# banyancomputer/hot-proofs-blake3-circom

Hardware: AMD Instinct MI355X
Metric: BLAKE3-compression witnesses/sec (higher is better)
Workload: dtype u32

## Files before the change

hot-proofs-blake3-circom_amd/build.py:

```python
import os, shutil, subprocess, sys

PKG = os.path.dirname(os.path.abspath(__file__))
ROOT = os.path.dirname(PKG)
CSRC = os.path.join(PKG, "csrc")
LIB = os.path.join(PKG, "libb3wit.so")
NAPI = os.path.join(PKG, "js", "b3wit_napi.node")
ARCH = "gfx950"


def _newer(target, sources):
    if not os.path.exists(target):
        return True
    t = os.path.getmtime(target)
    return any(os.path.getmtime(s) > t for s in sources)


def _run(cmd, **kw):
    print("+", " ".join(cmd), flush=True)
    subprocess.check_call(cmd, **kw)


def hipcc():
    for c in (os.environ.get("HIPCC"), shutil.which("hipcc"), "/opt/rocm/bin/hipcc"):
        if c and os.path.exists(c):
            return c
    raise RuntimeError("hipcc not found")


def build_lib(force=False, extra_flags=()):
    from concurrent.futures import ThreadPoolExecutor
    names = ("b3w_kernels.hip", "b3w_exact.hip", "b3w_plan.hip", "b3w_bao.hip", "b3w_placement.hip", "b3w_commit.hip", "b3w_r1cs.hip", "b3w_r1cs_walk.hip", "b3w_r1cs_host.cpp", "b3w_hostcomm.cpp",
             "b3w_ctx.cpp", "b3w_bodies.cpp", "b3w_wtns.cpp", "b3w_r1cs_api.cpp", "b3w_commit_api.cpp", "b3w_comm.cpp", "b3w_chain.cpp")
    srcs = [os.path.join(CSRC, f) for f in names]
    hdrs = [os.path.join(CSRC, f) for f in sorted(os.listdir(CSRC)) if f.endswith((".h", ".inc"))] + \
        [os.path.join(ROOT, "include", "b3wit.h")]
    objdir = os.path.join(PKG, "build")
    os.makedirs(objdir, exist_ok=True)
    if os.environ.get("B3W_BUILD_DIAG") == "1":
        extra_flags = (*extra_flags, "-DB3W_R1CS_DIAG")
    flags = [f"--offload-arch={ARCH}", "-O3", "-std=c++17", "-fPIC", "-x", "hip", "-Wall", "-Wno-unused-function", *extra_flags]
    jobs = []
    for src in srcs:
        obj = os.path.join(objdir, os.path.basename(src) + ".o")
        if force or extra_flags or _newer(obj, [src] + hdrs):
            jobs.append([hipcc(), *flags, "-c", src, "-o", obj])
    if jobs:
        with ThreadPoolExecutor(max_workers=min(len(jobs), os.cpu_count() or 1)) as ex:
            list(ex.map(_run, jobs))
    objs = [os.path.join(objdir, os.path.basename(src) + ".o") for src in srcs]
    if jobs or _newer(LIB, objs):
        _run([hipcc(), f"--offload-arch={ARCH}", "-fPIC", "-shared", "-o", LIB, *objs, "-ldl", "-lrt", "-lpthread"])
    return LIB


def build_oracle(force=False):
    so = os.path.join(ROOT, "oracle", "libb3w_oracle.so")
    if force or _newer(so, [os.path.join(ROOT, "oracle", "b3w_oracle.c")]):
        _run(["make", "-C", os.path.join(ROOT, "oracle")])
    return so


def build_napi(force=False):
    src = os.path.join(PKG, "js", "b3wit_napi.cc")
    if not os.path.exists(src):
        return None
    inc = "/usr/include/node"
    if not os.path.exists(os.path.join(inc, "node_api.h")):
        print("node_api.h not found; skipping N-API addon", file=sys.stderr)
        return None
    if force or _newer(NAPI, [src, os.path.join(ROOT, "include", "b3wit.h")]):
        _run(["g++", "-O2", "-std=c++17", "-fPIC", "-shared", "-DNODE_GYP_MODULE_NAME=b3wit_napi", "-I", inc,
              "-I", os.path.join(ROOT, "include"), "-o", NAPI, src, "-ldl"])
# ... 12 lines not shown
```

hot-proofs-blake3-circom_amd/csrc/b3w_ctx.cpp:

```cpp
#include "b3w_internal.h"
#include "b3w_layout_tables.inc"
#include "b3w_trace_tables.inc"

namespace {

struct Sha256 {
  uint32_t h[8];
  uint8_t buf[64];
  uint64_t len = 0;
  size_t fill = 0;
  Sha256() {
    static const uint32_t init[8] = {0x6a09e667, 0xbb67ae85, 0x3c6ef372, 0xa54ff53a, 0x510e527f, 0x9b05688c, 0x1f83d9ab, 0x5be0cd19};
    memcpy(h, init, sizeof h);
  }
  static uint32_t ror(uint32_t x, int r) { return (x >> r) | (x << (32 - r)); }
  void block(const uint8_t *p) {
    static const uint32_t K[64] = {
        0x428a2f98, 0x71374491, 0xb5c0fbcf, 0xe9b5dba5, 0x3956c25b, 0x59f111f1, 0x923f82a4, 0xab1c5ed5, 0xd807aa98, 0x12835b01,
        0x243185be, 0x550c7dc3, 0x72be5d74, 0x80deb1fe, 0x9bdc06a7, 0xc19bf174, 0xe49b69c1, 0xefbe4786, 0x0fc19dc6, 0x240ca1cc,
        0x2de92c6f, 0x4a7484aa, 0x5cb0a9dc, 0x76f988da, 0x983e5152, 0xa831c66d, 0xb00327c8, 0xbf597fc7, 0xc6e00bf3, 0xd5a79147,
        0x06ca6351, 0x14292967, 0x27b70a85, 0x2e1b2138, 0x4d2c6dfc, 0x53380d13, 0x650a7354, 0x766a0abb, 0x81c2c92e, 0x92722c85,
        0xa2bfe8a1, 0xa81a664b, 0xc24b8b70, 0xc76c51a3, 0xd192e819, 0xd6990624, 0xf40e3585, 0x106aa070, 0x19a4c116, 0x1e376c08,
        0x2748774c, 0x34b0bcb5, 0x391c0cb3, 0x4ed8aa4a, 0x5b9cca4f, 0x682e6ff3, 0x748f82ee, 0x78a5636f, 0x84c87814, 0x8cc70208,
        0x90befffa, 0xa4506ceb, 0xbef9a3f7, 0xc67178f2};
// ... 207 lines not shown
  return buf;
}

}

bool b3w_int_build_slot_table(const CircuitDesc &c, std::vector<uint32_t> &table, std::string &err) { return build_slot_table(c, table, err); }

namespace {
int32_t ensure_scratch(b3w_ctx *ctx) {
  if (ctx->d_scratch) return B3W_OK;
  ctx->scratch_cap = B3W_SWEEP_CHUNK;
  hipError_t e = hipMalloc((void **)&ctx->d_scratch, (size_t)ctx->scratch_cap * ctx->desc.lds_words * 4);
  if (e != hipSuccess) { ctx->scratch_cap = 0; return hip_fail(ctx, e, "hipMalloc(sweep scratch)"); }
  return B3W_OK;
}

void set_inputs(b3w_ctx *ctx) {
  struct Def { const char *name; uint32_t count; };
  static const Def comp[] = {{"h", 8}, {"m", 16}, {"t", 2}, {"b", 1}, {"d", 1}};
  static const Def nova[] = {{"n_blocks", 1}, {"block_count", 1}, {"h", 8}, {"chunk_idx_low", 1}, {"chunk_idx_high", 1},
                             {"leaf_depth", 1}, {"total_depth", 1}, {"depth", 1}, {"m", 16}, {"b", 1}};
  const Def *d = ctx->desc.kind == B3W_KIND_COMP ? comp : nova;
  const int nd = ctx->desc.kind == B3W_KIND_COMP ? 5 : 10;
  uint32_t off = 0;
  for (int i = 0; i < nd; i++) {
    ctx->inputs.push_back({d[i].name, d[i].count, off, fnv1a64(d[i].name)});
    off += d[i].count;
  }
}
}

int b3w_int_default_variant(const b3w_ctx *ctx, uint32_t n, const uint8_t *d_bodies, uint64_t pitch) {
  const bool comp = ctx->desc.kind == B3W_KIND_COMP, nova2 = ctx->desc.kind == B3W_KIND_NOVA_O2;
  const bool fillable = ctx->fill_ok && !(reinterpret_cast<uintptr_t>(d_bodies) & 31) && !(pitch & 31) && pitch < (1ull << 30) &&
                        (uint64_t)n * pitch + (1ull << 20) < (1ull << 37);
  if (fillable && comp && n >= 128 && (n <= 3072 || !b3w_place_is_mixed(d_bodies))) return B3W_VARIANT_REGIONFILL;
  if (fillable && nova2 && (b3w_place_is_mixed(d_bodies) ? n >= 768 && n <= 2560 : n >= 512)) return B3W_VARIANT_REGIONFILL;
  if (n <= 2560) return B3W_VARIANT_SLICED + (n <= (comp ? 32u : 8u) ? 64 : n <= 96 ? 32 : n <= 192 ? 16 : n <= 768 ? 8 : 4);
  if (comp) return n <= 6144 ? 0 : 8;
  if (nova2) return n <= 3072 ? 0 : n <= 32768 ? 3 : 4;
  return 0;
}

extern "C" {

uint32_t b3w_abi_version(void) { return (1u << 16) | 1u; }

int32_t b3w_identify_wasm(const uint8_t *code, size_t len) {
  if (!code) return B3W_CIRCUIT_UNKNOWN;
  Sha256 s;
  s.update(code, len);
  uint8_t dg[32];
  s.final(dg);
  char hex[65];
  for (int i = 0; i < 32; i++) snprintf(hex + 2 * i, 3, "%02x", dg[i]);
  for (int c = 0; c < 4; c++) if (!strcmp(hex, WASM_SHA256[c])) return c;
  return B3W_CIRCUIT_UNKNOWN;
}

int32_t b3w_create(int32_t circuit, int32_t device, b3w_ctx **out) {
  if (!out || circuit < 0 || circuit > 3) return B3W_E_BAD_ARGUMENT;
  *out = nullptr;
  int ndev = 0;
  if (hipGetDeviceCount(&ndev) != hipSuccess || ndev <= 0 || device < 0 || device >= ndev) return B3W_E_NO_DEVICE;
  b3w_ctx *ctx = new b3w_ctx;
  ctx->circuit = circuit;
  ctx->desc = CIRCUITS[circuit];
  ctx->device = device;
// ... 166 lines not shown
uint32_t b3w_public_words(const b3w_ctx *ctx) { return ctx ? ctx->desc.npub : 0; }

int32_t b3w_last_error(const b3w_ctx *ctx, char *buf, size_t len) {
  if (!ctx || !buf || !len) return B3W_E_BAD_ARGUMENT;
  snprintf(buf, len, "%s", ctx->last_error.c_str());
  return B3W_OK;
}

int32_t b3w_write_wtns_header(const b3w_ctx *ctx, uint8_t out[76]) {
  if (!ctx || !out) return B3W_E_BAD_ARGUMENT;
  uint32_t w[19];
  memcpy(&w[0], "wtns", 4);
  w[1] = 2; w[2] = 2;
  w[3] = 1; w[4] = 8 + 32; w[5] = 0;
  w[6] = 32;
  memcpy(&w[7], ctx->desc.prime, 32);
  w[15] = ctx->desc.nwit;
  const uint64_t len = 32ull * ctx->desc.nwit;
  w[16] = 2; w[17] = (uint32_t)len; w[18] = (uint32_t)(len >> 32);
  memcpy(out, w, 76);
  return B3W_OK;
}

int32_t b3w_batch_run_device(b3w_ctx *ctx, const uint32_t *d_records, uint32_t n, uint8_t *d_bodies, uint64_t pitch,
                             uint32_t *d_public, int32_t *d_status, void *stream) {
  if (!ctx || !d_records || !d_bodies) return B3W_E_BAD_ARGUMENT;
  const uint64_t body = 32ull * ctx->desc.nwit;
  if (pitch == 0) pitch = body;
  if (pitch < body || (pitch & 31)) { ctx->last_error = "pitch must be >= witness_size*32 and a multiple of 32"; return B3W_E_BAD_ARGUMENT; }
  if (reinterpret_cast<uintptr_t>(d_bodies) & 15) { ctx->last_error = "d_bodies must be 16-byte aligned"; return B3W_E_BAD_ARGUMENT; }
  ON_DEVICE(ctx);
  int variant = ctx->variant;
  if (ctx->variant_auto || (ctx->variant_tuned && n <= 2560)) variant = b3w_int_default_variant(ctx, n, d_bodies, pitch);
  if (variant >= B3W_VARIANT_REGIONFILL && !ctx->fill_ok) { ctx->last_error = "the fill-ordered variants (200, 201) exist for the compression circuit and the nova O2 builds"; return B3W_E_BAD_ARGUMENT; }
  int rc = b3w_launch_batch(ctx->desc.kind, variant, d_records, n, d_bodies, pitch, ctx->d_table, ctx->desc.nwit,
                            d_public, d_status, ctx->d_aux, ctx->d_scratch, ctx->scratch_cap, (hipStream_t)stream);
  if (rc == 0) return B3W_OK;
  if (rc == -5) { ctx->last_error = "the sweep and fill-ordered paths need 32-byte aligned bodies and pitch < 2^30"; return B3W_E_BAD_ARGUMENT; }
  if (rc < 0) { ctx->last_error = "no kernel for this circuit kind / variant"; return B3W_E_BAD_ARGUMENT; }
  return hip_fail(ctx, (hipError_t)rc, "kernel launch");
}

int32_t b3w_batch_verify_device(b3w_ctx *ctx, const uint8_t *d_bodies, uint32_t n, uint64_t pitch, uint32_t *d_mismatch,
                                void *stream) {
  if (!ctx || !d_bodies || !d_mismatch) return B3W_E_BAD_ARGUMENT;
  if (!ctx->d_in_slots) { ctx->last_error = "this circuit's layout does not keep every input as a slot"; return B3W_E_BAD_ARGUMENT; }
  const uint64_t body = 32ull * ctx->desc.nwit;
  if (pitch == 0) pitch = body;
  if (pitch < body || (pitch & 31) || (reinterpret_cast<uintptr_t>(d_bodies) & 15)) {
    ctx->last_error = "pitch must be >= witness_size*32 and a multiple of 32, bodies 16-byte aligned";
    return B3W_E_BAD_ARGUMENT;
  }
  ON_DEVICE(ctx);
  int rc = b3w_launch_verify(ctx->desc.kind, ctx->d_in_slots, n, d_bodies, pitch, ctx->d_table, ctx->desc.nwit, d_mismatch,
                             ctx->d_aux, (hipStream_t)stream);
  return rc ? hip_fail(ctx, (hipError_t)rc, "verify launch") : B3W_OK;
}

int32_t b3w_batch_autotune_device(b3w_ctx *ctx, const uint32_t *d_records, uint32_t n, uint8_t *d_bodies, uint64_t pitch,
                                  uint32_t *d_public, int32_t *d_status, void *stream, int32_t *chosen_variant,
                                  float *chosen_ms) {
  if (!ctx || !d_records || !d_bodies || !n) return B3W_E_BAD_ARGUMENT;
  ON_DEVICE(ctx);
  int32_t rc;
  if (n <= 2560 && (ctx->variant_auto || ctx->variant_tuned)) {
    float ms = 0;
    rc = B3W_OK;
    for (int w = 0; w < 2 && rc == B3W_OK; w++) rc = b3w_batch_run_device(ctx, d_records, n, d_bodies, pitch, d_public, d_status, stream);
    if (rc == B3W_OK) rc = b3w_batch_time_device(ctx, d_records, n, d_bodies, pitch, d_public, d_status, stream, 5, &ms);
    if (rc) return rc;
    if (chosen_variant) *chosen_variant = b3w_int_default_variant(ctx, n, d_bodies, pitch ? pitch : 32ull * ctx->desc.nwit);
    if (chosen_ms) *chosen_ms = ms;
    return B3W_OK;
  }
  rc = ensure_scratch(ctx);
  if (rc) return rc;
  const int candidates[6] = {0, ctx->desc.kind == B3W_KIND_COMP ? (n > 6144 ? 8 : 3) : ctx->desc.kind == B3W_KIND_NOVA_O2 ? 3 : 0, B3W_VARIANT_SWEEP,
                             ctx->fill_ok ? B3W_VARIANT_REGIONFILL : 0, ctx->desc.kind == B3W_KIND_NOVA_O2 && n >= 16384 ? 4 : 0,
                             ctx->fill_ok ? B3W_VARIANT_REGIONFILL_LIGHT : 0};
  int best = ctx->variant;
  float best_ms = 1e30f;
  const int saved = ctx->variant;
  const bool saved_auto = ctx->variant_auto;
  ctx->variant_auto = false;
  float cand_ms[6] = {1e30f, 1e30f, 1e30f, 1e30f, 1e30f, 1e30f};
  for (int round = 0; round < 2; round++) {
    for (int ci = 0; ci < 6; ci++) {
      const int c = candidates[ci];
      if (ci > 0 && c == candidates[0]) continue;
      if (round > 0 && cand_ms[ci] >= 1e30f) continue;
      ctx->variant = c;
      float ms = 0;
      rc = B3W_OK;
      for (int w = 0; w < 2 && rc == B3W_OK; w++)
        rc = b3w_batch_run_device(ctx, d_records, n, d_bodies, pitch, d_public, d_status, stream);
      if (rc == B3W_OK) rc = b3w_batch_time_device(ctx, d_records, n, d_bodies, pitch, d_public, d_status, stream, n <= 8192 ? 20 : 5, &ms);
      if (rc == B3W_E_BAD_ARGUMENT) continue;
      if (rc) { ctx->variant = saved; ctx->variant_auto = saved_auto; return rc; }
      if (ms < cand_ms[ci]) cand_ms[ci] = ms;
    }
  }
  for (int ci = 0; ci < 6; ci++)
    if (cand_ms[ci] < best_ms) { best_ms = cand_ms[ci]; best = candidates[ci]; }
  if (best_ms >= 1e30f) { ctx->variant = saved; ctx->variant_auto = saved_auto; return B3W_E_BAD_ARGUMENT; }
  ctx->variant = best;
  ctx->variant_tuned = true;
  if (chosen_variant) *chosen_variant = best;
  if (chosen_ms) *chosen_ms = best_ms;
  return B3W_OK;
}

int32_t b3w_batch_time_device(b3w_ctx *ctx, const uint32_t *d_records, uint32_t n, uint8_t *d_bodies, uint64_t pitch,
                              uint32_t *d_public, int32_t *d_status, void *stream, uint32_t iters, float *avg_ms) {
  if (!ctx || !avg_ms || !iters) return B3W_E_BAD_ARGUMENT;
  ON_DEVICE(ctx);
  hipEvent_t e0 = nullptr, e1 = nullptr;
  hipError_t e = hipEventCreate(&e0);
  if (e == hipSuccess) e = hipEventCreate(&e1);
  if (e == hipSuccess) e = hipEventRecord(e0, (hipStream_t)stream);
  int32_t rc = B3W_OK;
  for (uint32_t i = 0; i < iters && e == hipSuccess && rc == B3W_OK; i++)
    rc = b3w_batch_run_device(ctx, d_records, n, d_bodies, pitch, d_public, d_status, stream);
  float ms = 0;
  if (e == hipSuccess && rc == B3W_OK) e = hipEventRecord(e1, (hipStream_t)stream);
  if (e == hipSuccess && rc == B3W_OK) e = hipEventSynchronize(e1);
  if (e == hipSuccess && rc == B3W_OK) e = hipEventElapsedTime(&ms, e0, e1);
  if (e0) (void)hipEventDestroy(e0);
  if (e1) (void)hipEventDestroy(e1);
  if (rc) return rc;
  if (e != hipSuccess) return hip_fail(ctx, e, "timing events");
  *avg_ms = ms / iters;
  return B3W_OK;
}

static int32_t calc_witness_run(b3w_ctx *ctx, const std::vector<uint32_t> &rec, const std::vector<uint8_t> &fe, bool canonical,
                                uint8_t *out_body) {
  const CircuitDesc &d = ctx->desc;
// ... 70 lines not shown
```

hot-proofs-blake3-circom_amd/csrc/b3w_kernels.h:

```cpp
#pragma once
#include <hip/hip_runtime_api.h>
#include <stdint.h>

#define B3W_VARIANT_SWEEP 100
#define B3W_VARIANT_SLICED 20
#define B3W_VARIANT_REGIONFILL 200
#define B3W_VARIANT_REGIONFILL_LIGHT 201
#define B3W_REGIONFILL_GRID 256
#define B3W_AUX_WIDE_SLOTS (16 + 8 * 2048)
#define B3W_AUX_LINE_COUNTS (B3W_AUX_WIDE_SLOTS + 68)
#define B3W_AUX_LINE_LISTS (B3W_AUX_LINE_COUNTS + 4)
#define B3W_LINE_LIST_MAX 160
#define B3W_AUX_ALIAS_COUNT (B3W_AUX_LINE_LISTS + 2 * 4 * B3W_LINE_LIST_MAX)
#define B3W_AUX_ALIAS_LIST (B3W_AUX_ALIAS_COUNT + 1)
#define B3W_ALIAS_MAX 192
#define B3W_SWEEP_GRID 256
#define B3W_SWEEP_LOGC 13
#define B3W_SWEEP_CHUNK (1u << B3W_SWEEP_LOGC)

extern "C" int b3w_launch_batch(int kind, int variant, const uint32_t *d_recs, uint32_t n, uint8_t *d_out,
                                uint64_t pitch, const uint32_t *d_table, uint32_t nwit, uint32_t *d_pub,
                                int32_t *d_status, const void *d_aux, uint32_t *d_scratch, uint32_t scratch_cap,
                                hipStream_t stream);

extern "C" int b3w_launch_exact(int nova, const uint32_t *d_inputs, const uint32_t *d_prime, const uint32_t *d_table,
                                uint32_t nwit, uint8_t *d_out, uint32_t *d_status, hipStream_t stream);

extern "C" uint32_t b3w_plan_path_len(uint64_t chunk, uint64_t nchunks);
extern "C" int b3w_launch_plan_leaves(const uint8_t *d_pre, uint64_t total_len, uint64_t first_chunk, uint32_t nlocal,
                                      uint64_t nchunks, uint32_t *d_recs, uint32_t *d_chunk_cv, hipStream_t stream);
extern "C" int b3w_launch_plan_merge(const uint32_t *d_left, const uint32_t *d_right, uint32_t stride_words, uint64_t npairs,
                                     uint32_t root, uint32_t *d_parents, hipStream_t stream);
extern "C" int b3w_launch_plan_parents(const uint32_t *d_levels, uint64_t nchunks, uint64_t first_chunk, uint32_t nlocal,
                                       uint32_t last_chunk_blocks, uint32_t *d_recs, hipStream_t stream);
extern "C" uint32_t b3w_plan_tree_first_level(uint64_t nchunks);
extern "C" int b3w_launch_plan_tree(uint32_t *d_levels, uint64_t nchunks, uint32_t l0, uint32_t *d_root, uint64_t first_chunk, uint32_t plan_nlocal,
                                    uint32_t last_chunk_blocks, uint32_t *d_recs, hipStream_t stream);
extern "C" uint64_t b3w_plan_parent_row(uint64_t chunk, uint64_t nchunks);
extern "C" int b3w_plan_path_provable(uint64_t chunk, uint64_t nchunks);
extern "C" int b3w_launch_pack_hout(const uint32_t *d_pub, uint64_t row0, uint64_t count, uint32_t *d_dst, hipStream_t stream);
extern "C" int b3w_launch_unpack_hout(const uint32_t *d_gathered, uint64_t block_words, uint64_t par_off, const uint64_t *d_tab, uint32_t nranks,
                                      uint64_t max_rows, uint32_t *d_leaf_all, uint32_t *d_par_all, hipStream_t stream);

extern "C" int b3w_launch_trace(int kind, const uint32_t *d_recs, uint32_t cn, uint32_t *d_images, uint32_t row, const uint32_t *d_table,
                                uint32_t nwit, uint32_t *d_pub, int32_t *d_status, const void *d_aux, hipStream_t stream);
extern "C" int b3w_launch_verify(int kind, const uint32_t *d_in_slots, uint32_t n, const uint8_t *d_bodies, uint64_t pitch,
                                 const uint32_t *d_table, uint32_t nwit, uint32_t *d_mismatch, const void *d_aux,
                                 hipStream_t stream);

extern "C" int b3w_place_alloc(int device, uint64_t bytes, int want_mixed, void **out, int *mixed, float *rates);
extern "C" int b3w_place_free(void *ptr);
extern "C" int b3w_place_is_mixed(const void *ptr);
// ... 76 lines not shown
```

hot-proofs-blake3-circom_amd/csrc/b3w_kernels.hip:

```cpp
#include <hip/hip_runtime.h>
#include <stdint.h>
#include <stdlib.h>
#include <atomic>
#include "b3w_atoms.h"
#include "b3w_kernels.h"

namespace {

typedef uint32_t u32x4 __attribute__((ext_vector_type(4)));

__device__ __forceinline__ uint32_t rotr32(uint32_t x, int r) { return __builtin_rotateright32(x, r); }

template <int P0, int P1, int P2, int P3>
__device__ __forceinline__ uint32_t quad_perm(uint32_t x) {
  return (uint32_t)__builtin_amdgcn_update_dpp(0, (int)x, P0 | (P1 << 2) | (P2 << 4) | (P3 << 6), 0xF, 0xF, false);
}

__host__ __device__ constexpr uint64_t sched_pack(int r) {
  const int sigma[16] = {2, 6, 3, 10, 7, 0, 4, 13, 1, 11, 12, 5, 9, 14, 15, 8};
  int p[16] = {0, 1, 2, 3, 4, 5, 6, 7, 8, 9, 10, 11, 12, 13, 14, 15};
  for (int i = 0; i < r; i++) {
    int q[16] = {};
    for (int j = 0; j < 16; j++) q[j] = p[sigma[j]];
    for (int j = 0; j < 16; j++) p[j] = q[j];
  }
  uint64_t v = 0;
  for (int j = 0; j < 16; j++) v |= (uint64_t)p[j] << (4 * j);
  return v;
}

template <int R1, int R2>
__device__ __forceinline__ void half_g(uint32_t &a, uint32_t &b, uint32_t &c, uint32_t &d, uint32_t m,
                                       uint32_t *Lk) {
  const uint64_t s1 = (uint64_t)a + b + m;
  const uint32_t A = (uint32_t)s1;
// ... 824 lines not shown
  __builtin_amdgcn_fence(__ATOMIC_RELEASE, "wavefront");
  __builtin_amdgcn_wave_barrier();
}

#define B3W_RF_RING 256
struct RegionList {
  uint32_t n, body32, pitch32, off0, end;
  uint32_t grp, v_next, produced;
  int32_t zlo, zhi, xoff;
  bool done;
};
#define B3W_RF_STARTS 0x80000000u
#define B3W_RF_NEAR 0x40000000u
#define B3W_RF_REJECT 0x20000000u
#define B3W_RF_BODY 0x1FFFFFFFu
__device__ __forceinline__ void region_list_batch(RegionList &s, uint2 *ring, uint32_t lane) {
  const uint32_t v = s.v_next + lane, j = s.grp + 32u * v;
  const bool valid = (uint64_t)j << 12 < s.end;
  const uint32_t rs = j << 12, re = rs + 4096u;
  const uint32_t w_lo = (valid && rs >= s.off0 + s.body32) ? (rs - s.off0 - s.body32) / s.pitch32 + 1u : 0u;
  const uint32_t bs = s.off0 + w_lo * s.pitch32;
  const bool e1 = valid && w_lo < s.n && bs < re;
  const bool e2 = e1 && w_lo + 1 < s.n && bs + s.pitch32 < re;
  const uint64_t b1 = __builtin_amdgcn_ballot_w64(e1), b2 = __builtin_amdgcn_ballot_w64(e2), lt = (1ull << lane) - 1;
  const uint32_t pos = s.produced + __builtin_popcountll(b1 & lt) + __builtin_popcountll(b2 & lt);
  auto near = [&](int32_t rel) { const int32_t t = rel + s.xoff; return (t + 96 + 3072 + 35 > s.zlo && t < s.zhi + 4) ? B3W_RF_NEAR : 0u; };
  if (e1) ring[pos % B3W_RF_RING] = make_uint2(w_lo | (bs >= rs ? B3W_RF_STARTS : 0u) | near((int32_t)(rs - bs)), (uint32_t)((int32_t)(rs - bs) << 5));
  if (e2) ring[(pos + 1) % B3W_RF_RING] = make_uint2((w_lo + 1) | B3W_RF_STARTS | near((int32_t)(rs - bs - s.pitch32)), (uint32_t)((int32_t)(rs - bs - s.pitch32) << 5));
  s.produced = uni(s.produced + (uint32_t)__builtin_popcountll(b1) + (uint32_t)__builtin_popcountll(b2));
  s.v_next += 64;
  s.done = s.done || __builtin_amdgcn_ballot_w64(!valid) != 0;
}

template <int KIND, int NH>
__global__ __launch_bounds__(320, 1) void b3w_regionfill_kernel(const uint32_t *__restrict__ recs, uint32_t n,
                                                                uint8_t *__restrict__ out, uint64_t pitch,
                                                                const uint32_t *__restrict__ table, uint32_t nwit,
                                                                uint32_t *__restrict__ pub, int32_t *__restrict__ status, uint32_t pace,
                                                                const uint32_t *__restrict__ aux) {
  constexpr bool NOVA = KIND != B3W_KIND_COMP;
  constexpr int WORDS = NOVA ? B3W_LDS_WIDE : B3W_LDS_WORDS_COMP, NREC = NOVA ? 32 : 28, RDST = NOVA ? B3W_LDS_NV : B3W_A_H, R = 4;
  extern __shared__ __attribute__((aligned(16))) uint32_t bf_lds[];
  __shared__ uint2 ring[B3W_RF_RING];
  __shared__ uint32_t cnt_ring[4];
  uint16_t *tab = reinterpret_cast<uint16_t *>(bf_lds);
  const uint32_t tabw = ((nwit + 7u) & ~7u) / 2;
  uint32_t *lds = bf_lds + tabw;
  const uint32_t wave = uni(threadIdx.x >> 6), lane = threadIdx.x & 63u;
  const uint32_t x = blockIdx.x & 7u, grp = blockIdx.x >> 3;
  const uint32_t body = 32u * nwit;
  if (wave < 4) {
    const uint32_t padded = ((nwit + 31u) / 32u + 8u) * 32u;
    const uint4 *t8 = reinterpret_cast<const uint4 *>(table + padded);
    uint4 *tab8 = reinterpret_cast<uint4 *>(tab);
    const uint32_t n8 = (nwit + 7u) / 8u;
    for (uint32_t base8 = 0; base8 < n8; base8 += 256u * 4u) {
      uint4 v[4];
#pragma unroll
      for (int uu = 0; uu < 4; ++uu) {
        const uint32_t i8 = base8 + 256u * uu + threadIdx.x;
        v[uu] = i8 < n8 ? t8[i8] : make_uint4(0, 0, 0, 0);
      }
#pragma unroll
      for (int uu = 0; uu < 4; ++uu) {
        const uint32_t i8 = base8 + 256u * uu + threadIdx.x;
        if (i8 < n8) tab8[i8] = v[uu];
      }
    }
  }
  if (wave == 4) {
    const uint32_t q = lane >> 2, col = lane & 3;
    RegionList rl;
    rl.n = n; rl.body32 = nwit; rl.pitch32 = (uint32_t)(pitch >> 5);
    rl.off0 = (uint32_t)((reinterpret_cast<uint64_t>(out) & ((1ull << 17) - 1)) >> 5);
    rl.end = rl.off0 + (n - 1) * rl.pitch32 + rl.body32;
    rl.grp = grp; rl.v_next = 0; rl.produced = 0; rl.done = false;
    rl.xoff = (int32_t)(x << 7);
    rl.zlo = NOVA ? (int32_t)aux[B3W_AUX_WIDE_SLOTS] : 0x7FFFFFFF;
    rl.zhi = NOVA ? (int32_t)aux[B3W_AUX_WIDE_SLOTS + B3W_NOVA_ISZERO - 1] : -1;
    auto list_until = [&](uint32_t target) {
      while (!rl.done && rl.produced < target) region_list_batch(rl, ring, lane);
      __builtin_amdgcn_fence(__ATOMIC_RELEASE, "wavefront");
      __builtin_amdgcn_wave_barrier();
    };
    auto cnt_of = [&](uint32_t h) { return rl.produced <= h * NH ? 0u : (rl.produced - h * NH < (uint32_t)NH ? rl.produced - h * NH : (uint32_t)NH); };
    uint32_t al[3] = {0, 0, 0};
    if (NOVA) {
      const uint32_t na = aux[B3W_AUX_ALIAS_COUNT];
#pragma unroll
      for (int u = 0; u < 3; ++u) al[u] = lane + 64u * u < na ? aux[B3W_AUX_ALIAS_LIST + lane + 64u * u] : 0u;
    }
    TracerRecs<NH, NREC> tr;
    list_until(2 * NH);
    tracer_load<NH, NREC>(tr, recs, cnt_of(0), lane, [&](uint32_t k) { return ring[k % B3W_RF_RING].x & B3W_RF_BODY; });
    for (uint32_t h = 0;; ++h) {
      uint32_t *half = lds + (h & 1) * NH * WORDS;
      list_until((h + 3) * NH);
      const uint32_t cnt = cnt_of(h);
      if (lane == 0) cnt_ring[h & 3] = cnt;
      tracer_put<NH, NREC, WORDS, RDST>(tr, half, cnt, lane);
      tracer_load<NH, NREC>(tr, recs, cnt_of(h + 1), lane, [&](uint32_t k) { return ring[((h + 1) * NH + k) % B3W_RF_RING].x & B3W_RF_BODY; });
      if (!NOVA) {
        if (q < cnt) trace_compression(half + q * WORDS, col, nullptr);
      } else {
        if (q < cnt) {
          uint32_t *L = half + q * WORDS;
          const bool dom_a = nova_iszero_flags_quad(L, (int)col);
          const int32_t st = nova_select(L, (int)col, dom_a);
          if (col == 0) {
            L[B3W_LDS_OKWORD] = st == 0 ? 1u : 0u; L[B3W_LDS_STWORD] = (uint32_t)st;
            if (st != 0) ring[(h * NH + q) % B3W_RF_RING].x |= B3W_RF_REJECT;
          }
          if (st == 0) trace_compression(L, col, nullptr);
        }
        __builtin_amdgcn_fence(__ATOMIC_RELEASE, "wavefront");
        __builtin_amdgcn_wave_barrier();
        {
        uint32_t av[NH * 3];
#pragma unroll
        for (int qq = 0; qq < NH; ++qq)
#pragma unroll
          for (int u = 0; u < 3; ++u) av[qq * 3 + u] = ((uint32_t)qq < cnt && al[u]) ? half[qq * WORDS + (al[u] & 0xFFFFu)] : 0u;
#pragma unroll
        for (int qq = 0; qq < NH; ++qq)
#pragma unroll
          for (int u = 0; u < 3; ++u) if ((uint32_t)qq < cnt && al[u]) half[qq * WORDS + (al[u] >> 16)] = av[qq * 3 + u];
        }
      }
      __syncthreads();
      if (cnt < (uint32_t)NH) break;
    }
    return;
  }
  __builtin_amdgcn_s_setprio(3);
  const uint32_t par = lane & 1u;
  const uint32_t sub = wave;
  struct Ent { uint32_t wq; int32_t rel0, relw; uint32_t e[R]; };
  struct Wd { uint32_t w0[R], w1[R]; };
  auto s1 = [&](uint32_t k, Ent &en) {
    const uint2 d = ring[k % B3W_RF_RING];
    en.wq = uni(d.x);
    en.relw = (int32_t)uni(d.y) + (int32_t)((x << 12) + (sub << 10));
    en.rel0 = en.relw + (int32_t)(lane << 4);
    const int32_t s0 = en.rel0 >> 5;
    const uint16_t *tp = tab + s0;
#pragma unroll
    for (int r = 0; r < R; ++r) en.e[r] = tp[1024 * r];
  };
  auto s2 = [&](const Ent &en, Wd &wd, const uint32_t *img) {
#pragma unroll
    for (int r = 0; r < R; ++r) {
      const uint32_t *L = img + (en.e[r] & 0x3FFu);
      wd.w0[r] = L[0]; wd.w1[r] = L[1];
    }
  };
  auto s3 = [&](const Ent &en, const Wd &wd, const uint32_t *img) {
    if (NOVA || !(en.wq & B3W_RF_STARTS)) {
      for (uint32_t z = 0; z < (pace & 15u); ++z) __builtin_amdgcn_s_sleep(1);
      uint32_t pv = lane;
      for (uint32_t z = 0; z < (pace >> 4); ++z) asm volatile("v_add_u32 %0, %0, 1" : "+v"(pv));
    }
    const uint32_t w = en.wq & B3W_RF_BODY;
    if ((en.wq >> 31) && x == 0 && sub == 0) fill_report<NOVA>(img, w, lane, pub, status);
    uint8_t *dst = out + (uint64_t)w * pitch;
    if (NOVA) {
      const bool ok = !(en.wq & B3W_RF_REJECT);
      const __amdgpu_buffer_rsrc_t rsrc = __builtin_amdgcn_make_buffer_rsrc(dst, 0, (int)body, 0x00020000);
      if (en.wq & B3W_RF_NEAR) {
#pragma unroll
        for (int r = 0; r < R; ++r) fill_store_nova<true>(en.e[r], wd.w0[r], wd.w1[r], par, ok, rsrc, (uint32_t)(en.rel0 + (int32_t)(r << 15)), body, lane);
      } else {
#pragma unroll
        for (int r = 0; r < R; ++r) fill_store_nova<false>(en.e[r], wd.w0[r], wd.w1[r], par, ok, rsrc, (uint32_t)(en.rel0 + (int32_t)(r << 15)), body, lane);
      }
    } else {
#pragma unroll
      for (int r = 0; r < R; ++r) {
        const uint32_t rel = (uint32_t)(en.rel0 + (int32_t)(r << 15));
        fill_store<NOVA>(en.e[r], wd.w0[r], wd.w1[r], par, rel < body, dst + rel);
      }
    }
  };
  for (uint32_t h = 0;; ++h) {
    __syncthreads();
    const uint32_t cnt = uni(cnt_ring[h & 3]);
    const uint32_t *half = lds + (h & 1) * NH * WORDS;
    const uint32_t k0 = h * NH;
    Ent e0, e1, e2;
    Wd d0, d1, d2;
    if (0 < cnt) s1(k0, e0);
    if (1 < cnt) s1(k0 + 1, e1);
    if (0 < cnt) s2(e0, d0, half);
    for (uint32_t i = 0; i < cnt; i += 3) {
      if (i + 2 < cnt) s1(k0 + i + 2, e2);
      if (i + 1 < cnt) s2(e1, d1, half + (i + 1) * WORDS);
      s3(e0, d0, half + i * WORDS);
      if (i + 1 >= cnt) break;
      if (i + 3 < cnt) s1(k0 + i + 3, e0);
      if (i + 2 < cnt) s2(e2, d2, half + (i + 2) * WORDS);
      s3(e1, d1, half + (i + 1) * WORDS);
      if (i + 2 >= cnt) break;
      if (i + 4 < cnt) s1(k0 + i + 4, e1);
      if (i + 3 < cnt) s2(e0, d0, half + (i + 3) * WORDS);
      s3(e2, d2, half + (i + 2) * WORDS);
    }
    if (cnt < (uint32_t)NH) break;
  }
}

}

namespace {
template <bool WIDE, int K>
int launch_sweep(const uint32_t *d_images, uint32_t n, uint8_t *d_out, uint64_t pitch, const uint32_t *d_table,
                 uint32_t nwit, hipStream_t stream) {
  const uintptr_t addr = reinterpret_cast<uintptr_t>(d_out);
  if (pitch >= (1ull << 30) || (addr & 31)) return -5;
  const uint32_t lead = (uint32_t)(addr & 4095);
  static const int shape = getenv("B3W_SWEEP_SHAPE") ? atoi(getenv("B3W_SWEEP_SHAPE")) : 2;
  const size_t smem = (size_t)nwit * 4 + 16;
  constexpr size_t B3W_SWEEP_MAX_SMEM = 24614 * 4 + 16;
  if (smem > B3W_SWEEP_MAX_SMEM) return -5;
#define B3W_SWEEP_LAUNCH(PAIRS, SPLIT)                                                                              \
  {                                                                                                                 \
             \
    static std::atomic<uint64_t> attr_done{0};                                                                      \
    int dev = 0;                                                                                                    \
    (void)hipGetDevice(&dev);                                                                                       \
    const uint64_t bit = 1ull << (dev & 63);                                                                        \
    if (!(attr_done.load(std::memory_order_acquire) & bit)) {                                                       \
      hipError_t e = hipFuncSetAttribute(reinterpret_cast<const void *>(&b3w_sweep_kernel<WIDE, K, B3W_SWEEP_LOGC, PAIRS, SPLIT>), \
                                         hipFuncAttributeMaxDynamicSharedMemorySize, (int)B3W_SWEEP_MAX_SMEM);     \
      if (e != hipSuccess) return (int)e;                                                                           \
      attr_done.fetch_or(bit, std::memory_order_release);                                                           \
    }                                                                                                               \
    hipLaunchKernelGGL((b3w_sweep_kernel<WIDE, K, B3W_SWEEP_LOGC, PAIRS, SPLIT>), dim3(B3W_SWEEP_GRID), dim3(128 * PAIRS), smem, \
                       stream, d_images, n, d_out - lead, lead, (uint32_t)pitch, d_table, nwit);                    \
  }
  switch (shape) {
    case 1: B3W_SWEEP_LAUNCH(1, false); break;
// ... 14 lines not shown
  uint8_t *bodies = const_cast<uint8_t *>(d_bodies);
  const uint32_t pm = (uint32_t)(pitch >> 5) & 3u, stride = (pitch & 31) ? 1u : pm == 0 ? 1u : pm == 2 ? 2u : 4u;
#define B3W_VGRID(WV) dim3((n + stride * WV - 1) / (stride * WV) * stride)
  if (kind == B3W_KIND_COMP)
    hipLaunchKernelGGL((b3w_compression_kernel<4, false, 2>), B3W_VGRID(4), dim3(64), 0, stream, d_in_slots, n, bodies, pitch,
                       d_table, nwit, d_mismatch, (int32_t *)nullptr, stride);
  else if (kind == B3W_KIND_NOVA_O2)
    hipLaunchKernelGGL((b3w_nova_kernel<B3W_KIND_NOVA_O2, 2, false, 2>), B3W_VGRID(2), dim3(64), 0, stream, d_in_slots, n,
                       bodies, pitch, d_table, nwit, d_mismatch, (int32_t *)nullptr, (const uint32_t *)d_aux, stride);
  else
    hipLaunchKernelGGL((b3w_nova_kernel<B3W_KIND_NOVA_O1, 2, false, 2>), B3W_VGRID(2), dim3(64), 0, stream, d_in_slots, n,
                       bodies, pitch, d_table, nwit, d_mismatch, (int32_t *)nullptr, (const uint32_t *)d_aux, stride);
#undef B3W_VGRID
  return (int)hipGetLastError();
}

extern "C" int b3w_launch_trace(int kind, const uint32_t *d_recs, uint32_t cn, uint32_t *d_images, uint32_t row, const uint32_t *d_table,
                                uint32_t nwit, uint32_t *d_pub, int32_t *d_status, const void *d_aux, hipStream_t stream) {
  if (cn == 0) return 0;
  if (cn > row) return -4;
  if (kind == B3W_KIND_COMP)
    hipLaunchKernelGGL((b3w_compression_kernel<16, false, 1>), dim3((cn + 15) / 16), dim3(64), 0, stream, d_recs, cn,
                       reinterpret_cast<uint8_t *>(d_images), (uint64_t)row, d_table, nwit, d_pub, d_status, 1u);
  else if (kind == B3W_KIND_NOVA_O2)
    hipLaunchKernelGGL((b3w_nova_kernel<B3W_KIND_NOVA_O2, 4, false, 1>), dim3((cn + 3) / 4), dim3(64), 0, stream, d_recs, cn,
                       reinterpret_cast<uint8_t *>(d_images), (uint64_t)row, d_table, nwit, d_pub, d_status, (const uint32_t *)d_aux, 1u);
  else if (kind == B3W_KIND_NOVA_O1)
    hipLaunchKernelGGL((b3w_nova_kernel<B3W_KIND_NOVA_O1, 2, false, 1>), dim3((cn + 1) / 2), dim3(64), 0, stream, d_recs, cn,
                       reinterpret_cast<uint8_t *>(d_images), (uint64_t)row, d_table, nwit, d_pub, d_status, (const uint32_t *)d_aux, 1u);
  else return -2;
  return (int)hipGetLastError();
}

extern "C" int b3w_launch_batch(int kind, int variant, const uint32_t *d_recs, uint32_t n, uint8_t *d_out,
                                uint64_t pitch, const uint32_t *d_table, uint32_t nwit, uint32_t *d_pub,
                                int32_t *d_status, const void *d_aux, uint32_t *d_scratch, uint32_t scratch_cap,
                                hipStream_t stream) {
  if (n == 0) return 0;
  if (variant >= B3W_VARIANT_SWEEP && variant < B3W_VARIANT_REGIONFILL) {
    if (!d_scratch || scratch_cap != (1u << B3W_SWEEP_LOGC)) return -4;
    if (kind != B3W_KIND_COMP && !d_aux) return -3;
    uint32_t *d_images = d_scratch;
    for (uint32_t c0 = 0; c0 < n; c0 += scratch_cap) {
      const uint32_t cn = n - c0 < scratch_cap ? n - c0 : scratch_cap;
      uint32_t *pub_c = d_pub ? d_pub + (uint64_t)c0 * (kind == B3W_KIND_COMP ? 16 : 15) : nullptr;
      int32_t *st_c = d_status ? d_status + c0 : nullptr;
      uint8_t *out_c = d_out + (uint64_t)c0 * pitch;
      int rc = b3w_launch_trace(kind, d_recs + (uint64_t)c0 * (kind == B3W_KIND_COMP ? 28 : 32), cn, d_images, scratch_cap, d_table, nwit, pub_c,
                                st_c, d_aux, stream);
      if (rc) return rc;
      if (kind == B3W_KIND_COMP) rc = launch_sweep<false, 8>(d_images, cn, out_c, pitch, d_table, nwit, stream);
      else rc = launch_sweep<true, 4>(d_images, cn, out_c, pitch, d_table, nwit, stream);
      if (rc) return rc;
    }
    return (int)hipGetLastError();
  }
  if (variant == B3W_VARIANT_REGIONFILL || variant == B3W_VARIANT_REGIONFILL_LIGHT) {
    if (kind != B3W_KIND_COMP && kind != B3W_KIND_NOVA_O2) return -1;
    if (kind == B3W_KIND_NOVA_O2 && !d_aux) return -3;
    if ((reinterpret_cast<uintptr_t>(d_out) & 31) || (pitch & 31) || pitch >= (1ull << 30)) return -5;
    if (32ull * nwit < (1ull << 17) || (uint64_t)n * pitch + (1ull << 20) >= (1ull << 37)) return -5;
    constexpr int NH_C = 14, NH_N = 11;
    const bool nova = kind != B3W_KIND_COMP;
    const size_t smem = (size_t)((nwit + 7u) & ~7u) * 2 +
                        (size_t)(2 * (nova ? NH_N * B3W_LDS_WIDE : NH_C * B3W_LDS_WORDS_COMP) + 4) * 4;
    constexpr size_t B3W_FILL_MAX_SMEM = 160 * 1024 - 4096;
    if (smem > B3W_FILL_MAX_SMEM) return -5;
    static std::atomic<uint64_t> attr_done{0};
    int dev = 0;
    (void)hipGetDevice(&dev);
    const uint64_t bit = 1ull << (dev & 63);
    if (!(attr_done.load(std::memory_order_acquire) & bit)) {
      hipError_t e = hipFuncSetAttribute(reinterpret_cast<const void *>(&b3w_regionfill_kernel<B3W_KIND_COMP, NH_C>),
                                         hipFuncAttributeMaxDynamicSharedMemorySize, (int)B3W_FILL_MAX_SMEM);
      if (e == hipSuccess)
        e = hipFuncSetAttribute(reinterpret_cast<const void *>(&b3w_regionfill_kernel<B3W_KIND_NOVA_O2, NH_N>), hipFuncAttributeMaxDynamicSharedMemorySize,
                                (int)B3W_FILL_MAX_SMEM);
      if (e != hipSuccess) return (int)e;
      attr_done.fetch_or(bit, std::memory_order_release);
    }
    const char *pace_s = getenv("B3W_FILL_PACE");
    const int pace_env = pace_s ? atoi(pace_s) : -1;
    const uint32_t pace = pace_env >= 0 ? (uint32_t)pace_env : variant == B3W_VARIANT_REGIONFILL_LIGHT ? (nova ? 33u : 48u) : nova ? 18u : 33u;
    if (!nova) {
      hipLaunchKernelGGL((b3w_regionfill_kernel<B3W_KIND_COMP, NH_C>), dim3(B3W_REGIONFILL_GRID), dim3(320), smem, stream, d_recs, n, d_out, pitch,
                         d_table, nwit, d_pub, d_status, pace, (const uint32_t *)nullptr);
    } else {
      hipLaunchKernelGGL((b3w_regionfill_kernel<B3W_KIND_NOVA_O2, NH_N>), dim3(B3W_REGIONFILL_GRID), dim3(320), smem, stream, d_recs, n, d_out, pitch,
                         d_table, nwit, d_pub, d_status, pace, (const uint32_t *)d_aux);
      hipLaunchKernelGGL((b3w_nova_kernel<B3W_KIND_NOVA_O2, 2, false, 3>), dim3((n + 1) / 2), dim3(64), 0, stream, d_recs, n, d_out, pitch, d_table, nwit,
                         (uint32_t *)nullptr, (int32_t *)nullptr, (const uint32_t *)d_aux, 1u);
    }
    return (int)hipGetLastError();
  }
  if (variant > B3W_VARIANT_REGIONFILL_LIGHT) return -1;
  const uint32_t pm = (uint32_t)(pitch >> 5) & 3u, stride = (pitch & 31) ? 1u : pm == 0 ? 1u : pm == 2 ? 2u : 4u;
#define B3W_GRID(WV) dim3((n + stride * WV - 1) / (stride * WV) * stride)
  static const uint32_t lds_pad = getenv("B3W_LDS_PAD") ? (uint32_t)atoi(getenv("B3W_LDS_PAD")) : 0;
  if (kind == B3W_KIND_COMP) {
#define B3W_LAUNCH_COMP(WV, NTV)                                                                         \
  hipLaunchKernelGGL((b3w_compression_kernel<WV, NTV, 0>), B3W_GRID(WV), dim3(64), lds_pad, stream,        \
                     d_recs, n, d_out, pitch, d_table, nwit, d_pub, d_status, stride)
    if (variant >= B3W_VARIANT_SLICED && variant < B3W_VARIANT_SWEEP) {
      const uint32_t slices = (uint32_t)(variant - B3W_VARIANT_SLICED);
      if (slices < 2 || slices > 64) return -1;
      hipLaunchKernelGGL((b3w_compression_kernel<1, false, 0, true>), dim3(B3W_GRID(1).x * slices), dim3(64), 0, stream, d_recs, n, d_out,
                         pitch, d_table, nwit, d_pub, d_status, stride, slices);
      return (int)hipGetLastError();
    }
    switch (variant) {
      case 0: B3W_LAUNCH_COMP(4, false); break;
      case 1: B3W_LAUNCH_COMP(1, false); break;
      case 2: B3W_LAUNCH_COMP(2, false); break;
      case 3: B3W_LAUNCH_COMP(8, false); break;
      case 4: B3W_LAUNCH_COMP(4, true); break;
      case 5: B3W_LAUNCH_COMP(2, true); break;
      case 6: B3W_LAUNCH_COMP(1, true); break;
      case 7: B3W_LAUNCH_COMP(16, false); break;
      case 8:
        hipLaunchKernelGGL((b3w_compression_kernel<8, false, 0>), B3W_GRID(8), dim3(64), lds_pad ? lds_pad : 24576u, stream, d_recs, n, d_out,
                           pitch, d_table, nwit, d_pub, d_status, stride);
        break;
      default: return -1;
    }
#undef B3W_LAUNCH_COMP
// ... 44 lines not shown
```

Before: 9.295 million.

## Pace compression region-fill writes by realtime clock and widen table staging

For the compression circuit, the region-fill kernel now throttles its writer waves against a target rate measured with s_memrealtime deadlines, replacing fixed sleep and busy-add loops. The pace value is derived from a configured fill rate. The LDS table staging loop is also unrolled twelve-wide instead of four to issue more loads in flight. Other changes add a shared fits-check so tuned variants fall back when region-fill cannot run, and diagnostic timestamp hooks compiled only under a debug flag. The risks are that the rate constants are tuned to one machine and that the wider unroll raises register pressure.

```diff
diff --git a/hot-proofs-blake3-circom_amd/build.py b/hot-proofs-blake3-circom_amd/build.py
--- a/hot-proofs-blake3-circom_amd/build.py
+++ b/hot-proofs-blake3-circom_amd/build.py
@@ -37,7 +37,7 @@
     objdir = os.path.join(PKG, "build")
     os.makedirs(objdir, exist_ok=True)
     if os.environ.get("B3W_BUILD_DIAG") == "1":
-        extra_flags = (*extra_flags, "-DB3W_R1CS_DIAG")
+        extra_flags = (*extra_flags, "-DB3W_R1CS_DIAG", "-DB3W_FILL_DIAG")
     flags = [f"--offload-arch={ARCH}", "-O3", "-std=c++17", "-fPIC", "-x", "hip", "-Wall", "-Wno-unused-function", *extra_flags]
     jobs = []
     for src in srcs:
diff --git a/hot-proofs-blake3-circom_amd/csrc/b3w_ctx.cpp b/hot-proofs-blake3-circom_amd/csrc/b3w_ctx.cpp
--- a/hot-proofs-blake3-circom_amd/csrc/b3w_ctx.cpp
+++ b/hot-proofs-blake3-circom_amd/csrc/b3w_ctx.cpp
@@ -263,8 +263,7 @@
 
 int b3w_int_default_variant(const b3w_ctx *ctx, uint32_t n, const uint8_t *d_bodies, uint64_t pitch) {
   const bool comp = ctx->desc.kind == B3W_KIND_COMP, nova2 = ctx->desc.kind == B3W_KIND_NOVA_O2;
-  const bool fillable = ctx->fill_ok && !(reinterpret_cast<uintptr_t>(d_bodies) & 31) && !(pitch & 31) && pitch < (1ull << 30) &&
-                        (uint64_t)n * pitch + (1ull << 20) < (1ull << 37);
+  const bool fillable = ctx->fill_ok && b3w_fill_fits(ctx->desc.kind, n, d_bodies, pitch, ctx->desc.nwit);
   if (fillable && comp && n >= 128 && (n <= 3072 || !b3w_place_is_mixed(d_bodies))) return B3W_VARIANT_REGIONFILL;
   if (fillable && nova2 && (b3w_place_is_mixed(d_bodies) ? n >= 768 && n <= 2560 : n >= 512)) return B3W_VARIANT_REGIONFILL;
   if (n <= 2560) return B3W_VARIANT_SLICED + (n <= (comp ? 32u : 8u) ? 64 : n <= 96 ? 32 : n <= 192 ? 16 : n <= 768 ? 8 : 4);
@@ -497,6 +496,8 @@
   ON_DEVICE(ctx);
   int variant = ctx->variant;
   if (ctx->variant_auto || (ctx->variant_tuned && n <= 2560)) variant = b3w_int_default_variant(ctx, n, d_bodies, pitch);
+  if (ctx->variant_tuned && variant >= B3W_VARIANT_REGIONFILL && !b3w_fill_fits(ctx->desc.kind, n, d_bodies, pitch, ctx->desc.nwit))
+    variant = b3w_int_default_variant(ctx, n, d_bodies, pitch);
   if (variant >= B3W_VARIANT_REGIONFILL && !ctx->fill_ok) { ctx->last_error = "the fill-ordered variants (200, 201) exist for the compression circuit and the nova O2 builds"; return B3W_E_BAD_ARGUMENT; }
   int rc = b3w_launch_batch(ctx->desc.kind, variant, d_records, n, d_bodies, pitch, ctx->d_table, ctx->desc.nwit,
                             d_public, d_status, ctx->d_aux, ctx->d_scratch, ctx->scratch_cap, (hipStream_t)stream);
@@ -546,8 +547,9 @@
   int best = ctx->variant;
   float best_ms = 1e30f;
   const int saved = ctx->variant;
-  const bool saved_auto = ctx->variant_auto;
+  const bool saved_auto = ctx->variant_auto, saved_tuned = ctx->variant_tuned;
   ctx->variant_auto = false;
+  ctx->variant_tuned = false;
   float cand_ms[6] = {1e30f, 1e30f, 1e30f, 1e30f, 1e30f, 1e30f};
   for (int round = 0; round < 2; round++) {
     for (int ci = 0; ci < 6; ci++) {
@@ -561,13 +563,13 @@
         rc = b3w_batch_run_device(ctx, d_records, n, d_bodies, pitch, d_public, d_status, stream);
       if (rc == B3W_OK) rc = b3w_batch_time_device(ctx, d_records, n, d_bodies, pitch, d_public, d_status, stream, n <= 8192 ? 20 : 5, &ms);
       if (rc == B3W_E_BAD_ARGUMENT) continue;
-      if (rc) { ctx->variant = saved; ctx->variant_auto = saved_auto; return rc; }
+      if (rc) { ctx->variant = saved; ctx->variant_auto = saved_auto; ctx->variant_tuned = saved_tuned; return rc; }
       if (ms < cand_ms[ci]) cand_ms[ci] = ms;
     }
   }
   for (int ci = 0; ci < 6; ci++)
     if (cand_ms[ci] < best_ms) { best_ms = cand_ms[ci]; best = candidates[ci]; }
-  if (best_ms >= 1e30f) { ctx->variant = saved; ctx->variant_auto = saved_auto; return B3W_E_BAD_ARGUMENT; }
+  if (best_ms >= 1e30f) { ctx->variant = saved; ctx->variant_auto = saved_auto; ctx->variant_tuned = saved_tuned; return B3W_E_BAD_ARGUMENT; }
   ctx->variant = best;
   ctx->variant_tuned = true;
   if (chosen_variant) *chosen_variant = best;
diff --git a/hot-proofs-blake3-circom_amd/csrc/b3w_kernels.h b/hot-proofs-blake3-circom_amd/csrc/b3w_kernels.h
--- a/hot-proofs-blake3-circom_amd/csrc/b3w_kernels.h
+++ b/hot-proofs-blake3-circom_amd/csrc/b3w_kernels.h
@@ -7,6 +7,8 @@
 #define B3W_VARIANT_REGIONFILL 200
 #define B3W_VARIANT_REGIONFILL_LIGHT 201
 #define B3W_REGIONFILL_GRID 256
+#define B3W_FILL_RATE_200 7.28
+#define B3W_FILL_RATE_201 7.36
 #define B3W_AUX_WIDE_SLOTS (16 + 8 * 2048)
 #define B3W_AUX_LINE_COUNTS (B3W_AUX_WIDE_SLOTS + 68)
 #define B3W_AUX_LINE_LISTS (B3W_AUX_LINE_COUNTS + 4)
@@ -18,6 +20,7 @@
 #define B3W_SWEEP_LOGC 13
 #define B3W_SWEEP_CHUNK (1u << B3W_SWEEP_LOGC)
 
+extern "C" int b3w_fill_fits(int kind, uint32_t n, const void *d_out, uint64_t pitch, uint32_t nwit);
 extern "C" int b3w_launch_batch(int kind, int variant, const uint32_t *d_recs, uint32_t n, uint8_t *d_out,
                                 uint64_t pitch, const uint32_t *d_table, uint32_t nwit, uint32_t *d_pub,
                                 int32_t *d_status, const void *d_aux, uint32_t *d_scratch, uint32_t scratch_cap,
diff --git a/hot-proofs-blake3-circom_amd/csrc/b3w_kernels.hip b/hot-proofs-blake3-circom_amd/csrc/b3w_kernels.hip
--- a/hot-proofs-blake3-circom_amd/csrc/b3w_kernels.hip
+++ b/hot-proofs-blake3-circom_amd/csrc/b3w_kernels.hip
@@ -1,6 +1,7 @@
 #include <hip/hip_runtime.h>
 #include <stdint.h>
 #include <stdlib.h>
+#include <stdio.h>
 #include <atomic>
 #include "b3w_atoms.h"
 #include "b3w_kernels.h"
@@ -891,12 +892,21 @@
   s.done = s.done || __builtin_amdgcn_ballot_w64(!valid) != 0;
 }
 
+#define B3W_FILL_NSTAMP 8
+#ifdef B3W_FILL_DIAG
+#define B3W_FILL_STAMP(k, who)                                                                                        \
+  do {                                                                                                                \
+    if (stamps && (who) && lane == 0) stamps[blockIdx.x * B3W_FILL_NSTAMP + (k)] = (uint32_t)__builtin_amdgcn_s_memrealtime(); \
+  } while (0)
+#else
+#define B3W_FILL_STAMP(k, who) do {} while (0)
+#endif
 template <int KIND, int NH>
 __global__ __launch_bounds__(320, 1) void b3w_regionfill_kernel(const uint32_t *__restrict__ recs, uint32_t n,
                                                                 uint8_t *__restrict__ out, uint64_t pitch,
                                                                 const uint32_t *__restrict__ table, uint32_t nwit,
                                                                 uint32_t *__restrict__ pub, int32_t *__restrict__ status, uint32_t pace,
-                                                                const uint32_t *__restrict__ aux) {
+                                                                const uint32_t *__restrict__ aux, uint32_t *__restrict__ stamps) {
   constexpr bool NOVA = KIND != B3W_KIND_COMP;
   constexpr int WORDS = NOVA ? B3W_LDS_WIDE : B3W_LDS_WORDS_COMP, NREC = NOVA ? 32 : 28, RDST = NOVA ? B3W_LDS_NV : B3W_A_H, R = 4;
   extern __shared__ __attribute__((aligned(16))) uint32_t bf_lds[];
@@ -908,24 +918,27 @@
   const uint32_t wave = uni(threadIdx.x >> 6), lane = threadIdx.x & 63u;
   const uint32_t x = blockIdx.x & 7u, grp = blockIdx.x >> 3;
   const uint32_t body = 32u * nwit;
+  B3W_FILL_STAMP(0, wave == 0);
   if (wave < 4) {
+    constexpr uint32_t TL = 12;
     const uint32_t padded = ((nwit + 31u) / 32u + 8u) * 32u;
     const uint4 *t8 = reinterpret_cast<const uint4 *>(table + padded);
     uint4 *tab8 = reinterpret_cast<uint4 *>(tab);
     const uint32_t n8 = (nwit + 7u) / 8u;
-    for (uint32_t base8 = 0; base8 < n8; base8 += 256u * 4u) {
-      uint4 v[4];
-#pragma unroll
-      for (int uu = 0; uu < 4; ++uu) {
+    for (uint32_t base8 = 0; base8 < n8; base8 += 256u * TL) {
+      uint4 v[TL];
+#pragma unroll
+      for (uint32_t uu = 0; uu < TL; ++uu) {
         const uint32_t i8 = base8 + 256u * uu + threadIdx.x;
         v[uu] = i8 < n8 ? t8[i8] : make_uint4(0, 0, 0, 0);
       }
 #pragma unroll
-      for (int uu = 0; uu < 4; ++uu) {
+      for (uint32_t uu = 0; uu < TL; ++uu) {
         const uint32_t i8 = base8 + 256u * uu + threadIdx.x;
         if (i8 < n8) tab8[i8] = v[uu];
       }
     }
+    B3W_FILL_STAMP(1, wave == 0);
   }
   if (wave == 4) {
     const uint32_t q = lane >> 2, col = lane & 3;
@@ -951,6 +964,7 @@
     }
     TracerRecs<NH, NREC> tr;
     list_until(2 * NH);
+    B3W_FILL_STAMP(2, true);
     tracer_load<NH, NREC>(tr, recs, cnt_of(0), lane, [&](uint32_t k) { return ring[k % B3W_RF_RING].x & B3W_RF_BODY; });
     for (uint32_t h = 0;; ++h) {
       uint32_t *half = lds + (h & 1) * NH * WORDS;
@@ -958,6 +972,7 @@
       const uint32_t cnt = cnt_of(h);
       if (lane == 0) cnt_ring[h & 3] = cnt;
       tracer_put<NH, NREC, WORDS, RDST>(tr, half, cnt, lane);
+      B3W_FILL_STAMP(3, h == 0);
       tracer_load<NH, NREC>(tr, recs, cnt_of(h + 1), lane, [&](uint32_t k) { return ring[((h + 1) * NH + k) % B3W_RF_RING].x & B3W_RF_BODY; });
       if (!NOVA) {
         if (q < cnt) trace_compression(half + q * WORDS, col, nullptr);
@@ -986,14 +1001,18 @@
           for (int u = 0; u < 3; ++u) if ((uint32_t)qq < cnt && al[u]) half[qq * WORDS + (al[u] >> 16)] = av[qq * 3 + u];
         }
       }
+      B3W_FILL_STAMP(4, h == 0);
       __syncthreads();
       if (cnt < (uint32_t)NH) break;
     }
+    B3W_FILL_STAMP(7, true);
     return;
   }
   __builtin_amdgcn_s_setprio(3);
   const uint32_t par = lane & 1u;
   const uint32_t sub = wave;
+  uint32_t t1 = 0;
+  uint64_t due = 0;
   struct Ent { uint32_t wq; int32_t rel0, relw; uint32_t e[R]; };
   struct Wd { uint32_t w0[R], w1[R]; };
   auto s1 = [&](uint32_t k, Ent &en) {
@@ -1014,10 +1033,14 @@
     }
   };
   auto s3 = [&](const Ent &en, const Wd &wd, const uint32_t *img) {
-    if (NOVA || !(en.wq & B3W_RF_STARTS)) {
+    if (NOVA) {
       for (uint32_t z = 0; z < (pace & 15u); ++z) __builtin_amdgcn_s_sleep(1);
       uint32_t pv = lane;
       for (uint32_t z = 0; z < (pace >> 4); ++z) asm volatile("v_add_u32 %0, %0, 1" : "+v"(pv));
+    } else if (!(en.wq & B3W_RF_STARTS)) {
+      const uint32_t t_due = t1 + (uint32_t)(due >> 8);
+      while ((int32_t)((uint32_t)__builtin_amdgcn_s_memrealtime() - t_due) < 0) __builtin_amdgcn_s_sleep(1);
+      due += pace;
     }
     const uint32_t w = en.wq & B3W_RF_BODY;
     if ((en.wq >> 31) && x == 0 && sub == 0) fill_report<NOVA>(img, w, lane, pub, status);
@@ -1045,6 +1068,8 @@
     const uint32_t cnt = uni(cnt_ring[h & 3]);
     const uint32_t *half = lds + (h & 1) * NH * WORDS;
     const uint32_t k0 = h * NH;
+    if (!NOVA && h == 0) t1 = (uint32_t)__builtin_amdgcn_s_memrealtime();
+    B3W_FILL_STAMP(5, h == 0 && wave == 0);
     Ent e0, e1, e2;
     Wd d0, d1, d2;
     if (0 < cnt) s1(k0, e0);
@@ -1065,6 +1090,7 @@
     }
     if (cnt < (uint32_t)NH) break;
   }
+  B3W_FILL_STAMP(6, wave == 0);
 }
 
 }
@@ -1145,6 +1171,20 @@
   return (int)hipGetLastError();
 }
 
+#define B3W_FILL_NH_C 14
+#define B3W_FILL_NH_N 11
+static size_t fill_smem(int kind, uint32_t nwit) {
+  const bool nova = kind != B3W_KIND_COMP;
+  return (size_t)((nwit + 7u) & ~7u) * 2 + (size_t)(2 * (nova ? B3W_FILL_NH_N * B3W_LDS_WIDE : B3W_FILL_NH_C * B3W_LDS_WORDS_COMP) + 4) * 4;
+}
+constexpr size_t B3W_FILL_MAX_SMEM = 160 * 1024 - 4096;
+
+extern "C" int b3w_fill_fits(int kind, uint32_t n, const void *d_out, uint64_t pitch, uint32_t nwit) {
+  if ((reinterpret_cast<uintptr_t>(d_out) & 31) || (pitch & 31) || pitch >= (1ull << 30)) return 0;
+  if (32ull * nwit < (1ull << 17) || (uint64_t)n * pitch + (1ull << 20) >= (1ull << 37)) return 0;
+  return fill_smem(kind, nwit) <= B3W_FILL_MAX_SMEM;
+}
+
 extern "C" int b3w_launch_batch(int kind, int variant, const uint32_t *d_recs, uint32_t n, uint8_t *d_out,
                                 uint64_t pitch, const uint32_t *d_table, uint32_t nwit, uint32_t *d_pub,
                                 int32_t *d_status, const void *d_aux, uint32_t *d_scratch, uint32_t scratch_cap,
@@ -1171,14 +1211,10 @@
   if (variant == B3W_VARIANT_REGIONFILL || variant == B3W_VARIANT_REGIONFILL_LIGHT) {
     if (kind != B3W_KIND_COMP && kind != B3W_KIND_NOVA_O2) return -1;
     if (kind == B3W_KIND_NOVA_O2 && !d_aux) return -3;
-    if ((reinterpret_cast<uintptr_t>(d_out) & 31) || (pitch & 31) || pitch >= (1ull << 30)) return -5;
-    if (32ull * nwit < (1ull << 17) || (uint64_t)n * pitch + (1ull << 20) >= (1ull << 37)) return -5;
-    constexpr int NH_C = 14, NH_N = 11;
+    if (!b3w_fill_fits(kind, n, d_out, pitch, nwit)) return -5;
+    constexpr int NH_C = B3W_FILL_NH_C, NH_N = B3W_FILL_NH_N;
     const bool nova = kind != B3W_KIND_COMP;
-    const size_t smem = (size_t)((nwit + 7u) & ~7u) * 2 +
-                        (size_t)(2 * (nova ? NH_N * B3W_LDS_WIDE : NH_C * B3W_LDS_WORDS_COMP) + 4) * 4;
-    constexpr size_t B3W_FILL_MAX_SMEM = 160 * 1024 - 4096;
-    if (smem > B3W_FILL_MAX_SMEM) return -5;
+    const size_t smem = fill_smem(kind, nwit);
     static std::atomic<uint64_t> attr_done{0};
     int dev = 0;
     (void)hipGetDevice(&dev);
@@ -1192,18 +1228,45 @@
       if (e != hipSuccess) return (int)e;
       attr_done.fetch_or(bit, std::memory_order_release);
     }
+    uint32_t pace;
+    if (nova) {
+      pace = variant == B3W_VARIANT_REGIONFILL_LIGHT ? 33u : 18u;
+    } else {
+      const char *rate_s = getenv("B3W_FILL_RATE");
+      const double rate = rate_s && atof(rate_s) > 1.0 ? atof(rate_s) : variant == B3W_VARIANT_REGIONFILL_LIGHT ? B3W_FILL_RATE_201 : B3W_FILL_RATE_200;
+      pace = (uint32_t)(256.0 * (double)B3W_REGIONFILL_GRID * 16384.0 / (rate * 1e12) * 1e8 + 0.5);
+    }
     const char *pace_s = getenv("B3W_FILL_PACE");
-    const int pace_env = pace_s ? atoi(pace_s) : -1;
-    const uint32_t pace = pace_env >= 0 ? (uint32_t)pace_env : variant == B3W_VARIANT_REGIONFILL_LIGHT ? (nova ? 33u : 48u) : nova ? 18u : 33u;
+    if (pace_s && atoi(pace_s) >= 0) pace = (uint32_t)atoi(pace_s);
+    uint32_t *d_stamps = nullptr;
+#ifdef B3W_FILL_DIAG
+    static const char *stamp_path = getenv("B3W_FILL_STAMPS");
+    static uint32_t *stamp_buf = nullptr;
+    hipStreamCaptureStatus cap = hipStreamCaptureStatusNone;
+    (void)hipStreamIsCapturing(stream, &cap);
+    if (stamp_path && cap == hipStreamCaptureStatusNone) {
+      if (!stamp_buf && hipMalloc((void **)&stamp_buf, B3W_REGIONFILL_GRID * B3W_FILL_NSTAMP * 4) != hipSuccess) stamp_buf = nullptr;
+      d_stamps = stamp_buf;
+      if (d_stamps) (void)hipMemsetAsync(d_stamps, 0, B3W_REGIONFILL_GRID * B3W_FILL_NSTAMP * 4, stream);
+    }
+#endif
     if (!nova) {
       hipLaunchKernelGGL((b3w_regionfill_kernel<B3W_KIND_COMP, NH_C>), dim3(B3W_REGIONFILL_GRID), dim3(320), smem, stream, d_recs, n, d_out, pitch,
-                         d_table, nwit, d_pub, d_status, pace, (const uint32_t *)nullptr);
+                         d_table, nwit, d_pub, d_status, pace, (const uint32_t *)nullptr, d_stamps);
     } else {
       hipLaunchKernelGGL((b3w_regionfill_kernel<B3W_KIND_NOVA_O2, NH_N>), dim3(B3W_REGIONFILL_GRID), dim3(320), smem, stream, d_recs, n, d_out, pitch,
-                         d_table, nwit, d_pub, d_status, pace, (const uint32_t *)d_aux);
+                         d_table, nwit, d_pub, d_status, pace, (const uint32_t *)d_aux, d_stamps);
       hipLaunchKernelGGL((b3w_nova_kernel<B3W_KIND_NOVA_O2, 2, false, 3>), dim3((n + 1) / 2), dim3(64), 0, stream, d_recs, n, d_out, pitch, d_table, nwit,
                          (uint32_t *)nullptr, (int32_t *)nullptr, (const uint32_t *)d_aux, 1u);
     }
+#ifdef B3W_FILL_DIAG
+    if (d_stamps) {
+      uint32_t h_st[B3W_REGIONFILL_GRID * B3W_FILL_NSTAMP];
+      if (hipMemcpyAsync(h_st, d_stamps, sizeof h_st, hipMemcpyDeviceToHost, stream) == hipSuccess && hipStreamSynchronize(stream) == hipSuccess) {
+        if (FILE *f = fopen(stamp_path, "ab")) { fwrite(h_st, sizeof h_st, 1, f); fclose(f); }
+      }
+    }
+#endif
     return (int)hipGetLastError();
   }
   if (variant > B3W_VARIANT_REGIONFILL_LIGHT) return -1;
```

New measurement: 9.361 million (median of 6 runs). About the same (+0.7%).
